# google/data-driven-discretization-1d

Hardware: AMD Instinct MI355X
Metric: grid-point-steps/s (higher is better)
Workload: dtype f32

## Files before the change

data-driven-discretization-1d_amd/csrc/rhs_mfma.h:

```cpp
#pragma once
#include <type_traits>
#include <utility>

#include "dev_params.h"
#include "mfma_layout.h"

namespace ddd {
namespace mfma {

constexpr int kHS = 36;
constexpr int kTrigMax = 12;
__host__ __device__ constexpr int tab_rows(bool wide) { return wide ? 4 : 4 + flavour_channels(false); }

typedef float f32x16 __attribute__((ext_vector_type(16)));
typedef float f32x4 __attribute__((ext_vector_type(4)));
typedef float f32x2 __attribute__((ext_vector_type(2)));

template <int kK_, int kCB_>
struct Tower {
  static constexpr int kK = kK_;
  static constexpr int kCB = kCB_;
  static constexpr int kC = 32 * kCB_;
  static constexpr int kHS = kC + 4;
  static constexpr int kInSteps = (kK_ + 2) / 2;
// ... 255 lines not shown
  const float t = __builtin_amdgcn_exp2f(ax * -2.885390081777927f);
  const float q = (1.0f - t) * __builtin_amdgcn_rcpf(1.0f + t);
  const float x2 = x * x;
  const float poly =
      ax * fmaf(x2, fmaf(x2, fmaf(x2, fmaf(x2, 62.0f / 2835.0f, -17.0f / 315.0f), 2.0f / 15.0f),
                         -1.0f / 3.0f), 1.0f);
  return copysignf(ax < 0.25f ? poly : q, x);
}

__device__ __forceinline__ void activate16(f32x16& acc, int act) {
  if (act == ACT_RELU) {
#pragma unroll
    for (int r = 0; r < 16; r += 2) {
      f32x2 v{acc[r], acc[r + 1]}, y;
      asm("v_pk_add_f32 %0, %1, 0 clamp" : "=v"(y) : "v"(v));
      acc[r] = y[0];
      acc[r + 1] = y[1];
    }
  } else if (act == ACT_RELU6) {
#pragma unroll
    for (int r = 0; r < 16; ++r) acc[r] = fminf(fmaxf(acc[r], 0.0f), 6.0f);
  } else if (act == ACT_TANH) {
#pragma unroll
    for (int r = 0; r < 16; ++r) acc[r] = fast_tanh(acc[r]);
  } else if (act == ACT_SOFTPLUS) {
#pragma unroll
    for (int r = 0; r < 16; ++r) acc[r] = apply_activation(acc[r], ACT_SOFTPLUS);
  } else if (act == ACT_ELU) {
#pragma unroll
    for (int r = 0; r < 16; ++r) acc[r] = apply_activation(acc[r], ACT_ELU);
  }
}

__device__ __forceinline__ void store_tile32(float* out, int trow, int half,
                                             const f32x16& acc) {
  float* orow = out + trow * kHS + 4 * half;
#pragma unroll
  for (int qd = 0; qd < 4; ++qd)
    *reinterpret_cast<float4*>(orow + 8 * qd) = make_float4(
        acc[4 * qd + 0], acc[4 * qd + 1], acc[4 * qd + 2], acc[4 * qd + 3]);
}

__device__ __forceinline__ void store_tile32_at_bytes(float* out, int byte_off, const f32x16& acc) {
  char* orow = reinterpret_cast<char*>(out) + byte_off;
#pragma unroll
  for (int qd = 0; qd < 4; ++qd)
    *reinterpret_cast<float4*>(orow + 32 * qd) = make_float4(
        acc[4 * qd + 0], acc[4 * qd + 1], acc[4 * qd + 2], acc[4 * qd + 3]);
}

__device__ __forceinline__ float upper_half_one(float x) {
  return __builtin_amdgcn_inverse_ballot_w64(0xffffffff00000000ull) ? 1.0f : x;
}

template <int kWR, bool kShfl, bool kAddr = false>
__device__ __forceinline__ void input_layer(const DevParams& p, const Lane& ln,
                                            const float* __restrict__ us, float un,
                                            float* __restrict__ out,
                                            const float (&w)[kInSteps],
                                            const int (&rows)[2][kKW], int act,
                                            const int (*bperm)[3] = nullptr, int st_off = 0) {
  constexpr int kT = kWR / 32;
  const int j = ln.lane & 31;
  const int half = ln.lane >> 5;
  f32x16 acc[kT];
  float b0[kT], b1[kT], b2[kT];
#pragma unroll
  for (int t = 0; t < kT; ++t) {
    if (kAddr && kShfl) {
      const int uni = __float_as_int(un);
      b0[t] = __int_as_float(__builtin_amdgcn_ds_bpermute(bperm[t][0], uni));
      b1[t] = __int_as_float(__builtin_amdgcn_ds_bpermute(bperm[t][1], uni));
      b2[t] = __int_as_float(__builtin_amdgcn_ds_bpermute(bperm[t][2], uni));
    } else if (kAddr) {
      const char* __restrict__ ub = reinterpret_cast<const char*>(us);
      b0[t] = *reinterpret_cast<const float*>(ub + bperm[t][0]);
      b1[t] = *reinterpret_cast<const float*>(ub + bperm[t][1]);
      b2[t] = *reinterpret_cast<const float*>(ub + bperm[t][2]);
    } else {
      const int r0 = half ? rows[t][1] : rows[t][0];
      const int r1 = half ? rows[t][3] : rows[t][2];
      const int r2 = rows[t][4];
      b0[t] = kShfl ? __shfl(un, r0, 64) : us[r0];
      b1[t] = kShfl ? __shfl(un, r1, 64) : us[r1];
      b2[t] = kShfl ? __shfl(un, r2, 64) : us[r2];
    }
    b2[t] = kAddr ? upper_half_one(b2[t]) : (half ? 1.0f : b2[t]);
  }
  if (kAddr && kShfl) __builtin_amdgcn_sched_group_barrier(0x080, 3 * kT, 0);
#pragma unroll
  for (int t = 0; t < kT; ++t) {
#pragma unroll
    for (int r = 0; r < 16; ++r) acc[t][r] = 0.0f;
  }
#pragma unroll
  for (int t = 0; t < kT; ++t) acc[t] = DDD_MFMA32(w[0], b0[t], acc[t]);
#pragma unroll
  for (int t = 0; t < kT; ++t) acc[t] = DDD_MFMA32(w[1], b1[t], acc[t]);
#pragma unroll
  for (int t = 0; t < kT; ++t) acc[t] = DDD_MFMA32(w[2], b2[t], acc[t]);
#pragma unroll
  for (int t = 0; t < kT; ++t) {
    activate16(acc[t], act);
    if (kAddr) store_tile32_at_bytes(out, st_off + t * 32 * kHS * 4, acc[t]);
    else store_tile32(out, ln.wave * kWR + t * 32 + j, half, acc[t]);
  }
}

template <int kWR, bool kByteOffsets = false, int kPrio = 0>
__device__ __forceinline__ void hidden_layer(const DevParams& p, const Lane& ln,
                                             const float* __restrict__ in,
                                             float* __restrict__ out,
                                             const float (&w)[kHidSteps],
                                             const int (&rows)[2][kKW], int act, int st_off = 0) {
  constexpr int kT = kWR / 32;
  const int j = ln.lane & 31;
  const int half = ln.lane >> 5;
  int rowo[kT][kKW];
#pragma unroll
  for (int t = 0; t < kT; ++t)
#pragma unroll
    for (int tap = 0; tap < kKW; ++tap)
      rowo[t][tap] = kByteOffsets ? rows[t][tap]
                                  : (int)__umul24((unsigned)rows[t][tap], (unsigned)(kHS * 4)) +
                                        64 * half;
  const auto operand = [&](int t, int tap, int q) {
    return *reinterpret_cast<const float4*>(reinterpret_cast<const char*>(in) + rowo[t][tap] + 16 * q);
  };
  f32x16 acc[kT];
  float4 cur[kT], nxt[kT];
#pragma unroll
  for (int t = 0; t < kT; ++t) {
#pragma unroll
    for (int r = 0; r < 16; ++r) acc[t][r] = 0.0f;
    cur[t] = operand(t, 0, 0);
  }
  __builtin_amdgcn_sched_group_barrier(0x100, kT, 0);
#pragma unroll
  for (int g = 0; g < 20; ++g) {
    if (kPrio == 5 && g == 1) __builtin_amdgcn_s_setprio(0);
    if (kPrio == 5 && g == 19) __builtin_amdgcn_s_setprio(3);
#pragma unroll
    for (int t = 0; t < kT; ++t) {
      nxt[t] = cur[t];
      if (g + 1 < 20) nxt[t] = operand(t, (g + 1) >> 2, (g + 1) & 3);
    }
#pragma unroll
    for (int t = 0; t < kT; ++t) acc[t] = DDD_MFMA32(w[4 * g + 0], cur[t].x, acc[t]);
#pragma unroll
    for (int t = 0; t < kT; ++t) acc[t] = DDD_MFMA32(w[4 * g + 1], cur[t].y, acc[t]);
#pragma unroll
    for (int t = 0; t < kT; ++t) acc[t] = DDD_MFMA32(w[4 * g + 2], cur[t].z, acc[t]);
#pragma unroll
    for (int t = 0; t < kT; ++t) acc[t] = DDD_MFMA32(w[4 * g + 3], cur[t].w, acc[t]);
#pragma unroll
    for (int t = 0; t < kT; ++t) cur[t] = nxt[t];
    __builtin_amdgcn_sched_group_barrier(0x100, kT, 0);
    __builtin_amdgcn_sched_group_barrier(0x008, 4 * kT, 0);
  }
#pragma unroll
  for (int t = 0; t < kT; ++t) {
    acc[t] = DDD_MFMA32(w[80], 1.0f, acc[t]);
  }
#pragma unroll
  for (int t = 0; t < kT; ++t) {
    activate16(acc[t], act);
    if (kByteOffsets) store_tile32_at_bytes(out, st_off + t * 32 * kHS * 4, acc[t]);
    else store_tile32(out, ln.wave * kWR + t * 32 + j, half, acc[t]);
  }
}

#define DDD_MFMA16(A, B, C) __builtin_amdgcn_mfma_f32_16x16x4f32((A), (B), (C), 0, 0, 0)
__host__ __device__ constexpr int quad_channel_float(int c) {
  return 4 * (4 * (c >> 4) + (c & 3)) + ((c & 15) >> 2);
}

__device__ __forceinline__ void activate4(f32x4& acc, int act) {
  if (act == ACT_RELU) {
#pragma unroll
    for (int r = 0; r < 4; r += 2) {
      f32x2 v{acc[r], acc[r + 1]}, y;
      asm("v_pk_add_f32 %0, %1, 0 clamp" : "=v"(y) : "v"(v));
      acc[r] = y[0];
      acc[r + 1] = y[1];
    }
  } else {
#pragma unroll
    for (int r = 0; r < 4; ++r) acc[r] = apply_activation(acc[r], act);
  }
}

__device__ __forceinline__ void store_tile16(float* out, int st_off, const f32x4& acc) {
  char* o = reinterpret_cast<char*>(out) + st_off;
#pragma unroll
  for (int r = 0; r < 4; ++r) *reinterpret_cast<float*>(o + 16 * r) = acc[r];
// ... 457 lines not shown
  }
#pragma unroll
  for (int h = 0; h < kCB; ++h)
#pragma unroll
    for (int t = 0; t < kT; ++t) acc[h][t] = DDD_MFMA32(wb[h], 1.0f, acc[h][t]);
#pragma unroll
  for (int h = 0; h < kCB; ++h)
#pragma unroll
    for (int t = 0; t < kT; ++t) {
      activate16(acc[h][t], act);
      store_tile32_at<TW::kHS>(out, ln.wave * kWR + t * 32 + j, h, half, acc[h][t]);
    }
}

template <int kAbid>
__device__ __forceinline__ f32x4 mfma4(float a, float b, f32x4 c) {
  return __builtin_amdgcn_mfma_f32_4x4x1f32(a, b, c, 4, kAbid, 0);
}

template <int NG, int Q0, int NW, int kAcc, int... J>
__device__ __forceinline__ void fin4_mfmas(const float (&w)[NW], const f32x4& b,
                                           f32x4 (&acc)[kAcc], std::integer_sequence<int, J...>) {
  ((acc[J % kAcc] = mfma4<(Q0 + J) % 16>(w[(Q0 + J) / 16], b[J / NG], acc[J % kAcc])), ...);
}

template <int NG>
__device__ __forceinline__ void load_final4(const DevParams& p, int lane,
                                            float (&w)[fin4_regs(NG)]) {
  load_rows4<fin4_regs(NG)>(p.w_final4, lane, w);
}

constexpr int kFin4Ahead = 2;

template <int NG, int OG, class TW, int kAcc>
__device__ __forceinline__ void fin4_step(const char* __restrict__ in, const int (&off)[TW::kK],
                                          const float (&w)[fin4_regs_t<TW>(NG)],
                                          f32x4 (&buf)[kFin4Ahead + 1], f32x4 (&acc)[kAcc]) {
  constexpr int kNext = OG + kFin4Ahead;
  constexpr int kPerTap = TW::kFinC / 4;
  if constexpr (kNext < TW::kOperandGroups)
    buf[kNext % (kFin4Ahead + 1)] =
        *reinterpret_cast<const f32x4*>(in + off[kNext / kPerTap] + 16 * (kNext % kPerTap));
  fin4_mfmas<NG, OG * 4 * NG, fin4_regs_t<TW>(NG), kAcc>(w, buf[OG % (kFin4Ahead + 1)], acc,
                                                         std::make_integer_sequence<int, 4 * NG>{});
  if constexpr (kNext < TW::kOperandGroups) __builtin_amdgcn_sched_group_barrier(0x100, 1, 0);
  __builtin_amdgcn_sched_group_barrier(0x008, 4 * NG, 0);
}

template <int NG, class TW, int kAcc, int... OG>
__device__ __forceinline__ void fin4_run(const char* __restrict__ in, const int (&off)[TW::kK],
                                         const float (&w)[fin4_regs_t<TW>(NG)],
                                         f32x4 (&buf)[kFin4Ahead + 1], f32x4 (&acc)[kAcc],
                                         std::integer_sequence<int, OG...>) {
  (fin4_step<NG, OG, TW, kAcc>(in, off, w, buf, acc), ...);
}

template <int NG, class TW = DefaultTower, int kAcc = NG, int kPrio = 0>
__device__ __forceinline__ void final_layer4(const float* __restrict__ in_f,
                                             const float (&w)[fin4_regs_t<TW>(NG)],
                                             const int (&off)[TW::kK], f32x4 (&acc)[kAcc]) {
  const char* __restrict__ in = reinterpret_cast<const char*>(in_f);
  constexpr int kPerTap = TW::kFinC / 4;
  f32x4 buf[kFin4Ahead + 1];
#pragma unroll
  for (int g = 0; g < kAcc; ++g) acc[g] = f32x4{0.0f, 0.0f, 0.0f, 0.0f};
#pragma unroll
  for (int og = 0; og < kFin4Ahead; ++og)
    buf[og] = *reinterpret_cast<const f32x4*>(in + off[og / kPerTap] + 16 * (og % kPerTap));
  __builtin_amdgcn_sched_group_barrier(0x100, kFin4Ahead, 0);
  if (kPrio == 5) __builtin_amdgcn_s_setprio(1);
  fin4_run<NG, TW, kAcc>(in, off, w, buf, acc, std::make_integer_sequence<int, TW::kOperandGroups>{});
  if (kPrio == 5) __builtin_amdgcn_s_setprio(3);
  fin4_mfmas<NG, (TW::kFinK - 1) * NG, fin4_regs_t<TW>(NG), kAcc>(
      w, f32x4{1.0f, 1.0f, 1.0f, 1.0f}, acc, std::make_integer_sequence<int, NG>{});
}

template <int NG, int kPrio = 0>
__device__ __forceinline__ void final_layer4_t16(const float* __restrict__ in_f,
                                                 const float (&w)[fin4_regs_t<Tile16Tower>(NG)],
                                                 const int (&off)[kKW], f32x4 (&acc)[NG]) {
  const char* __restrict__ in = reinterpret_cast<const char*>(in_f);
  f32x4 cur[4], nxt[4];
#pragma unroll
  for (int g = 0; g < NG; ++g) acc[g] = f32x4{0.0f, 0.0f, 0.0f, 0.0f};
#pragma unroll
  for (int q = 0; q < 4; ++q) cur[q] = *reinterpret_cast<const f32x4*>(in + off[0] + 16 * q);
  __builtin_amdgcn_sched_group_barrier(0x100, 4, 0);
  if (kPrio == 5) __builtin_amdgcn_s_setprio(1);
  constexpr int kNW = fin4_regs_t<Tile16Tower>(NG);
  const auto tap_steps = [&](auto tap_c) {
    constexpr int tap = decltype(tap_c)::value;
#pragma unroll
    for (int q = 0; q < 4; ++q) {
      nxt[q] = cur[q];
      if (tap + 1 < kKW) nxt[q] = *reinterpret_cast<const f32x4*>(in + off[tap + 1 < kKW ? tap + 1 : tap] + 16 * q);
    }
    fin4_mfmas<NG, (4 * tap + 0) * 4 * NG, kNW, NG>(w, f32x4{cur[0][0], cur[1][0], cur[2][0], cur[3][0]}, acc,
                                                 std::make_integer_sequence<int, 4 * NG>{});
    fin4_mfmas<NG, (4 * tap + 1) * 4 * NG, kNW, NG>(w, f32x4{cur[0][1], cur[1][1], cur[2][1], cur[3][1]}, acc,
                                                 std::make_integer_sequence<int, 4 * NG>{});
    fin4_mfmas<NG, (4 * tap + 2) * 4 * NG, kNW, NG>(w, f32x4{cur[0][2], cur[1][2], cur[2][2], cur[3][2]}, acc,
                                                 std::make_integer_sequence<int, 4 * NG>{});
    fin4_mfmas<NG, (4 * tap + 3) * 4 * NG, kNW, NG>(w, f32x4{cur[0][3], cur[1][3], cur[2][3], cur[3][3]}, acc,
                                                 std::make_integer_sequence<int, 4 * NG>{});
// ... 74 lines not shown
__device__ __forceinline__ void forcing_phase1(const DevParams& p, Shared<kRows, kWR, kWide, TW>& sm,
                                               const Resident& res, float t, int tid) {
  if (tid < res.frc_pairs) {
    float sn, cs;
    sincos_branchless(res.frc_omega * t + res.frc_phi, &sn, &cs);
    sm.pm[tid] = make_float2(res.frc_a * sn, res.frc_a * cs);
  }
}

template <int kRows, int kWR, bool kMasked = false, bool kWide = false, class TW = DefaultTower>
__device__ __forceinline__ float forcing_phase2(Shared<kRows, kWR, kWide, TW>& sm, const Resident& res) {
  const int cnt = (res.frc_run >> 16) & 0xff;
  const float* __restrict__ pm = reinterpret_cast<const float*>(sm.pm) + (res.frc_run & 0xffff);
  float acc = 0.0f;
  int first = 0;
  if (kMasked) {
    float v[8];
#pragma unroll
    for (int i = 0; i < 8; ++i) v[i] = pm[2 * i];
#pragma unroll
    for (int i = 0; i < 8; ++i) acc = fmaf(v[i], res.frc_mask[i], acc);
    first = 8;
  }
  for (int m = first; m < cnt; m += 8) {
    float v[8];
#pragma unroll
    for (int i = 0; i < 8; ++i) v[i] = pm[2 * (m + i)];
#pragma unroll
    for (int i = 0; i < 8; ++i) acc = acc + (m + i < cnt ? v[i] : 0.0f);
  }
  return acc;
}

template <int kRows, int kWR, bool kMasked = false, bool kWide = false, class TW = DefaultTower>
__device__ __forceinline__ float forcing_sums(const DevParams& p, Shared<kRows, kWR, kWide, TW>& sm,
                                              const Resident& res, float t, int tid) {
  forcing_phase1<kRows, kWR>(p, sm, res, t, tid);
  group_barrier<kRows, kWR>();
  return forcing_phase2<kRows, kWR, kMasked>(sm, res);
}

template <int kRows, int kWR, bool kHoist, int kEq, bool kTrace, bool kWide, class TW = DefaultTower>
__device__ __forceinline__ float eval_rhs(const DevParams& p, Shared<kRows, kWR, kWide, TW>& sm, int batch,
                                          float u, float t, float t_next, Resident& res,
                                          bool fast_forcing, float* derivs_out,
                                          float* coeffs_out, bool prepare_next = true,
                                          int group = -1, int ablate = 0,
                                          unsigned long long* trace = nullptr) {
#define DDD_STAMP(i) do { if (kTrace && trace != nullptr && group_tid<kRows, kWR>() == 0) trace[i] = __builtin_amdgcn_s_memtime(); } while (0)
  DDD_STAMP(0);
  constexpr bool kSpec = kEq >= 0;
  const int eqn = kSpec ? kEq : p.equation;
  const int nD = kSpec ? spec_derivs(kEq) : opaque_scalar(p.D);
  const int nG = kSpec ? spec_stencil(kEq) : opaque_scalar(p.G);
  const unsigned dsel_valid = kSpec ? 0u : (unsigned)opaque_scalar((int)p.dsel_valid);
  const unsigned long long dsel_bits = kSpec ? 0ull : opaque_scalar(p.dsel_bits);
  const int rt_groups = kSpec ? 0 : opaque_scalar(p.rt_groups);
  const bool flux_form = kSpec ? spec_flux_form(kEq) : (p.conservative != 0);
  const bool fixed = kSpec ? false : (p.fixed != 0 || p.linear_taps != 0);
  const bool folded = kSpec ? spec_folded(kSpec ? kEq : 0) : (p.folded != 0);
  const int target = kSpec ? (int)TARGET_COEFFICIENTS : p.target;
  const int act = kSpec ? (int)ACT_RELU : p.act;
  const bool forced = kSpec ? (spec_forced_family(kSpec ? kEq : 0) && p.forced != 0)
                            : (p.forced != 0);
  if (kSpec) fast_forcing = true;
  const int nL = kHoist ? 3 : p.L;
  const bool pow2 = kRows == 64 || (p.N & (p.N - 1)) == 0;
  constexpr bool kOneWave = kRows == kWR;
  constexpr int kPrio = prio_mode(kEq);
  constexpr int kNG = kSpec ? spec_fin_groups(kSpec ? kEq : 0) : 2;
  constexpr int kGW = flavour_stencil(kWide);
  constexpr int kCh = flavour_net_channels(kWide);
  static_assert(!(kSpec && kWide), "the per-equation kernels have no wide flavour");
  static_assert(TW::kDefault || (!kSpec && !kWide && !kHoist && kWR == 64),
                "towers other than 5 taps x 32 channels: run-time-parameterised kernels only");
  constexpr bool kSplit = kSpec && kRows == 64 && kWR == 32 && kHoist;
  constexpr bool kQuad = kSpec && kRows == 64 && kWR == 16 && kHoist;
  static_assert(kWR != 16 || kQuad, "16-row wavefronts: per-equation integrators only");
  constexpr bool kKeepOffsets = (kWR == 64 || kSplit || kQuad) && kHoist;
  constexpr bool kKeepRows = kKeepOffsets && kEq >= 0;
  constexpr bool kKeepPatch = kKeepOffsets && !kWide;
  const int tid = opaque(group_tid<kRows, kWR>());
  const Lane ln = make_lane<kRows, kWR>(p, batch, tid, group < 0 ? (int)blockIdx.x : group);
  if (ln.owner) sm.u[ln.row] = u;
  const bool clamps_nan = !fixed && (act == ACT_RELU || act == ACT_RELU6);
  if (clamps_nan && !kOneWave) {
    if (__builtin_amdgcn_ballot_w64(u != u) != 0 && ln.lane == 0) sm.nan_flag = 1;
  }
  const auto nan_in_receptive_field = [&]() -> bool {
    const int n = p.N, lk = p.K >> 1;
    int span = p.L * (p.K - 1);
    span = span < n - 1 ? span : n - 1;
    int q = (ln.pos - p.L * lk) % n;
    q = q < 0 ? q + n : q;
    bool hit = false;
    for (int i = 0; i <= span; ++i) {
      const float v = sm.u[ln.base + q];
      hit = hit || (v != v);
      q = q + 1 == n ? 0 : q + 1;
    }
    return hit;
  };
  int hid_rows[2][TW::kK];
  if (!fixed && !kQuad) {
    if constexpr (!TW::kDefault) {
#pragma unroll
      for (int t2 = 0; t2 < 2; ++t2)
        tap_rows_n<TW>(ln, ln.wave * kWR + t2 * 32 + (ln.lane & 31), p.N, pow2, hid_rows[t2]);
    } else if constexpr (kKeepOffsets) {
#pragma unroll
      for (int t2 = 0; t2 < 2; ++t2)
#pragma unroll
        for (int k = 0; k < kKW; ++k) hid_rows[t2][k] = res.hid_off[t2][k];
    } else {
// ... 2 lines not shown
        tap_rows<kRows == 64>(ln, ln.wave * kWR + t2 * 32 + (ln.lane & 31), p.N, hid_rows[t2]);
    }
  }
  const float q_un = u * p.inv_stddev;
  float un_reg = fmaf(fmaf(-q_un, p.stddev, u), p.inv_stddev, q_un);
  if (p.exact_div) {
    asm volatile("; exact division");
    un_reg = u / p.stddev;
  }
  if (!fixed && !kOneWave && ln.owner) sm.un[ln.row] = un_reg;
  group_barrier<kRows, kWR>();
  const bool trig_lds = p.n_k <= 4;
  if (forced && fast_forcing && res.frc_slot >= 0)
    sm.fk[res.frc_slot] = res.fk_next;

  bool nan_any = false, poisoned = false;
  if (clamps_nan && !kOneWave) {
    nan_any = __builtin_amdgcn_readfirstlane(sm.nan_flag) != 0;
    if (nan_any) poisoned = nan_in_receptive_field();
  }
  float pch[kGW];
  const int gl = nG >> 1;
  if (!kOneWave) {
#pragma unroll
    for (int g = 0; g < kGW; ++g)
      pch[g] = (g < nG) ? sm.u[kKeepPatch ? res.pch_idx[g < kGMax ? g : 0]
                               : pow2 ? (((ln.pos + g - gl) & (p.N - 1)) | ln.base)
                                      : wrap_row(ln.base, ln.pos, g - gl, p.N)] : 0.0f;
  }

  float net[kCh];
#pragma unroll
  for (int c = 0; c < kCh; ++c) net[c] = 0.0f;
  if (!fixed) {
    DDD_STAMP(1);
    if (kPrio) __builtin_amdgcn_s_setprio(kPrio == 2 ? 0 : 3);
    if constexpr (TW::kDefault && !kQuad) {
      if (!kHoist && nL > 2) load_hidden(p, 0, ln.lane, res.hid);
    }
    if constexpr (kQuad) {
      input_layer_quad(sm.un, sm.hA, res.q_in, res.q_in_off, res.q_st_off, act, ln.lane);
    } else if constexpr (TW::kTile16) {
      static_assert(kKeepOffsets && kWR == 64 && kOneWave, "16-channel tiles: resident one-wave integrators");
      input_layer_t16(un_reg, sm.hA, res.w_in, res.t16_in_perm, res.t16_st_off, act, ln.lane);
    } else if constexpr (!TW::kDefault) {
      input_layer_big<TW, kWR, kOneWave>(p, ln, sm.un, un_reg, sm.hA, hid_rows, act);
    } else if (!(ablate & 16)) {
      input_layer<kWR, kOneWave, kKeepOffsets>(p, ln, sm.un, un_reg, sm.hA, res.w_in, hid_rows,
                                               act, res.in_perm, res.st_off);
    }
    const bool frc_next = forced && fast_forcing && prepare_next && !(ablate & 1);
    if (frc_next) forcing_phase1<kRows, kWR>(p, sm, res, t_next, tid);
    float* in = sm.hA;
    float* out = Shared<kRows, kWR, kWide, TW>::kSingleBuffer ? sm.hA : sm.hB;
    for (int l = 1; l < nL - 1; ++l) {
      if constexpr (kQuad) {
        group_barrier<kRows, kWR>();
        hidden_layer_quad(in, out, res.q_hid, res.q_hid_off, res.q_st_off, act);
      } else if constexpr (!TW::kDefault) {
        group_barrier<kRows, kWR>();
        if constexpr (TW::kRolled)
          hidden_layer_rolled<TW, kWR>(p, ln, l - 1, in, out, p.N, pow2, act);
        else if (l == 1 && res.hw_valid)
          hidden_layer_stream<TW, kWR, resident_groups<TW>()>(p, ln, 0, in, out, hid_rows, act,
                                                              res.hw, res.hwb);
        else
          hidden_layer_stream<TW, kWR>(p, ln, l - 1, in, out, hid_rows, act);
      } else {
        if (!kHoist && l > 1) load_hidden(p, l - 1, ln.lane, res.hid);
        group_barrier<kRows, kWR>();
        if constexpr (TW::kTile16) {
          hidden_layer_t16<kPrio>(in, out, res.hid, res.t16_hid_off, res.t16_st_off, act);
        } else {
          hidden_layer<kWR, kKeepOffsets, kPrio>(p, ln, in, out, res.hid, hid_rows, act, res.st_off);
        }
      }
      float* tmp = in; in = out; out = tmp;
    }
    DDD_STAMP(2);
    {
      if constexpr (kQuad) {
        constexpr bool kMaskedSums = spec_folded(kSpec ? kEq : 0);
        if (frc_next) res.fk_next = forcing_phase2<kRows, kWR, kMaskedSums>(sm, res);
        group_barrier<kRows, kWR>();
        const f32x4 d4 = final_layer_quad(in, res.q_fin, res.q_fin_off);
        *reinterpret_cast<float4*>(reinterpret_cast<char*>(out) + res.q_xch_off) =
            make_float4(d4[0], d4[1], d4[2], d4[3]);
        asm volatile("s_waitcnt lgkmcnt(0)" ::: "memory");
        const float* mine = out + ln.row * kHS;
#pragma unroll
        for (int g4 = 0; g4 < kNG; ++g4) {
          const float4 v = *reinterpret_cast<const float4*>(mine + 4 * g4);
          net[4 * g4] = v.x; net[4 * g4 + 1] = v.y; net[4 * g4 + 2] = v.z; net[4 * g4 + 3] = v.w;
        }
      } else if constexpr (kSplit) {
        constexpr int kNA = (kNG + 1) / 2, kNB = kNG - kNA;
        constexpr bool kMaskedSums = spec_folded(kSpec ? kEq : 0);
        if (frc_next) res.fk_next = forcing_phase2<kRows, kWR, kMaskedSums>(sm, res);
        group_barrier<kRows, kWR>();
        int off4[kKW];
#pragma unroll
        for (int k = 0; k < kKW; ++k) off4[k] = res.fin4_off[k];
        float* xch = out + ln.lane * kHS;
        if (ln.wave == 0) {
          float wa[fin4_regs(kNA)];
#pragma unroll
          for (int s2 = 0; s2 < fin4_regs(kNA); ++s2) wa[s2] = res.w_fin4[s2];
// ... 26 lines not shown
      float wf4[kFirstRows];
      if (!kKeepRows) {
        if constexpr (kSpec) {
          load_rows4<kFirstRows>(p.w_final4, opaque(ln.lane), wf4);
        } else {
          const float* __restrict__ wsrc = p.w_final4_rt + opaque(ln.lane);
#pragma unroll
          for (int s2 = 0; s2 < kFirstRows; ++s2) wf4[s2] = wsrc[s2 * 64];
        }
      }
      int off4[TW::kK];
      if constexpr (kKeepRows) {
#pragma unroll
        for (int s2 = 0; s2 < kFirstRows; ++s2) wf4[s2] = res.w_fin4[s2];
      }
      if constexpr (!TW::kDefault) {
        int rows_k[TW::kK];
        tap_rows_n<TW>(ln, ln.row, p.N, pow2, rows_k);
#pragma unroll
        for (int k = 0; k < TW::kK; ++k)
          off4[k] = (int)__umul24((unsigned)rows_k[k], (unsigned)(TW::kHS * 4));
      } else if constexpr (kKeepOffsets) {
#pragma unroll
        for (int k = 0; k < kKW; ++k) off4[k] = res.fin4_off[k];
      } else {
        int rows5[kKW];
        tap_rows<kRows == 64>(ln, ln.row, p.N, rows5);
#pragma unroll
        for (int k = 0; k < kKW; ++k)
          off4[k] = (int)__umul24((unsigned)rows5[k], (unsigned)(kHS * 4));
      }
      if (nL == 2) group_barrier<kRows, kWR>();
      constexpr bool kMaskedSums = kKeepRows && spec_folded(kSpec ? kEq : 0);
      if (frc_next) res.fk_next = forcing_phase2<kRows, kWR, kMaskedSums>(sm, res);
      group_barrier<kRows, kWR>();
      if constexpr (kSpec) {
        f32x4 acc4[kNG];
        if (!(ablate & 4)) {
          if constexpr (TW::kTile16) final_layer4_t16<kNG, kPrio>(in, wf4, off4, acc4);
          else final_layer4<kNG, TW, kNG, kPrio>(in, wf4, off4, acc4);
        } else {
#pragma unroll
          for (int g4 = 0; g4 < kNG; ++g4) acc4[g4] = f32x4{0.0f, 0.0f, 0.0f, 0.0f};
        }
#pragma unroll
        for (int g4 = 0; g4 < kNG; ++g4)
#pragma unroll
          for (int r4 = 0; r4 < 4; ++r4) net[4 * g4 + r4] = acc4[g4][r4];
      } else if constexpr (!kSpec) {
        constexpr int kPairRows = fin4_regs_t<TW>(2);
        const int head = rt_head_groups(rt_groups);
        int done = 0;
        if (!(ablate & 4)) {
          float wnext[kPairRows];
          const auto fetch_pair = [&](int first_group) {
            const float* __restrict__ wn = p.w_final4_rt +
                (size_t)(fin4_regs_t<TW>(head) + (first_group - head) / 2 * kPairRows) * 64 +
                opaque(ln.lane);
#pragma unroll
            for (int s2 = 0; s2 < kPairRows; ++s2) wnext[s2] = wn[s2 * 64];
          };
          if (head > 0 && head < rt_groups) fetch_pair(head);
          if (head == 3) {
            f32x4 acc3[3];
            final_layer4<3, TW>(in, wf4, off4, acc3);
#pragma unroll
            for (int g4 = 0; g4 < 3; ++g4)
#pragma unroll
              for (int r4 = 0; r4 < 4; ++r4) net[4 * g4 + r4] = acc3[g4][r4];
          } else if (head == 1) {
            float w1[fin4_regs_t<TW>(1)];
#pragma unroll
            for (int s2 = 0; s2 < fin4_regs_t<TW>(1); ++s2) w1[s2] = wf4[s2];
            f32x4 acc1[2];
            final_layer4<1, TW, 2>(in, w1, off4, acc1);
#pragma unroll
// ... 42 lines not shown
    if (forced && fast_forcing && prepare_next && !(ablate & 1))
      res.fk_next = forcing_sums<kRows, kWR>(p, sm, res, t_next, tid);
    group_barrier<kRows, kWR>();
  }

  if (clamps_nan) {
    if (kOneWave) {
      nan_any = __builtin_amdgcn_ballot_w64(u != u) != 0;
      if (nan_any) poisoned = nan_in_receptive_field();
    }
    if (nan_any) {
      const float qnan = __int_as_float(0x7fc00000);
#pragma unroll
      for (int c = 0; c < kCh; ++c) net[c] = poisoned ? qnan : net[c];
    }
  }
  float4 trig4[kTrigMax / 4];
  if (forced && fast_forcing) {
    if (kKeepOffsets) {
#pragma unroll
      for (int i = 0; i < kTrigMax / 4; ++i) trig4[i] = res.trig[i];
    } else if (trig_lds) {
      trig4[0] = *reinterpret_cast<const float4*>(sm.hA + ln.row * TW::kHS + TW::kC);
      trig4[1] = *reinterpret_cast<const float4*>(
          sm.hB + ln.row * Shared<kRows, kWR, kWide, TW>::kHBStride + Shared<kRows, kWR, kWide, TW>::kHBPad);
      trig4[2] = make_float4(0.0f, 0.0f, 0.0f, 0.0f);
    } else {
      const float4* __restrict__ tr =
          reinterpret_cast<const float4*>(p.trig) + (size_t)opaque(ln.pos) * (kTrigMax / 4);
#pragma unroll
      for (int i = 0; i < kTrigMax / 4; ++i) trig4[i] = tr[i];
    }
  }
  if (kOneWave) {
#pragma unroll
    for (int g = 0; g < kGW; ++g)
      pch[g] = (g < nG) ? sm.u[kKeepPatch ? res.pch_idx[g < kGMax ? g : 0]
                               : pow2 ? (((ln.pos + g - gl) & (p.N - 1)) | ln.base)
                                      : wrap_row(ln.base, ln.pos, g - gl, p.N)] : 0.0f;
  }
  f32x2 cf2[kMaxDerivs][kGW / 2];
#define CF(d, g) cf2[d][(g) >> 1][(g) & 1]
#pragma unroll
  for (int d = 0; d < kMaxDerivs; ++d)
#pragma unroll
    for (int q = 0; q < kGW / 2; ++q) cf2[d][q] = f32x2{0.0f, 0.0f};
  if (kWide) {
    if (!fixed && target == TARGET_COEFFICIENTS) {
      const auto take = [&](auto slot_c) {
        constexpr int kSlot = decltype(slot_c)::value;
#pragma unroll
        for (int d = 0; d < kWideDerivs; ++d)
#pragma unroll
          for (int g = 0; g < kSlot; ++g)
            if (kSlot * d + g < kCh && g < kGW) CF(d, g) = net[(kSlot * d + g) % kCh];
      };
      if (nG <= kGMax) take(std::integral_constant<int, kGMax>{});
      else if (nG == 9) take(std::integral_constant<int, 9>{});
      else if (nG == 10) take(std::integral_constant<int, 10>{});
      else if (nG == 11) take(std::integral_constant<int, 11>{});
      else take(std::integral_constant<int, 12>{});
    }
  } else if (!fixed && folded) {
    if (kSpec) {
#pragma unroll
      for (int g = 0; g < kGW; ++g)
        if (g < nG) { CF(0, g) = net[g]; CF(1, g) = net[nG + g]; }
// ... 104 lines not shown
          s = fmaf(CF(d, g), pch[g], s);
          asm("" : "+v"(s));
        }
      dv[d] = s;
    }
  }
  if (derivs_out != nullptr && ln.active) {
#pragma unroll
    for (int d = 0; d < kMaxDerivs; ++d)
      if (d < nD) derivs_out[(size_t)ln.gidx * nD + d] = dv[d];
  }

  float r = equation_rhs_or_flux(eqn, u, dv, p.eta);
  const bool direct_time = !kSpec && !fixed && target == TARGET_TIME_DERIVATIVE;
  const bool direct_flux = !kSpec && !fixed && target == TARGET_FLUX;
  if (direct_time || direct_flux) r = net[0];
  if ((flux_form && !direct_time) || direct_flux) {
    float fnext;
    if (kOneWave) {
      if (p.N == 64 && p.dpp_rol)
        fnext = ops::wave_rotate_left1(r);
      else
        fnext = __shfl(r, pow2 ? (((ln.pos + 1) & (p.N - 1)) | ln.base)
                                    : wrap_row(ln.base, ln.pos, 1, p.N), 64);
    } else {
      if (ln.owner) sm.flux[ln.row] = r;
      group_barrier<kRows, kWR>();
      fnext = sm.flux[wrap_row(ln.base, ln.pos, 1, p.N)];
    }
    r = p.inv_dx * (fnext - r);
    if (!direct_flux) r = -r;
  }
  if (forced && !(ablate & 1)) {
    if (kSpec || fast_forcing) {
      const float4* __restrict__ fk4 =
          kKeepOffsets ? reinterpret_cast<const float4*>(reinterpret_cast<const char*>(sm.fk) + res.fk_off)
                       : reinterpret_cast<const float4*>(sm.fk + ln.sl * kTrigMax);
      float total = 0.0f;
#pragma unroll
      for (int i = 0; i < kTrigMax / 4; ++i) {
        if (i == 2 && trig_lds && !kKeepOffsets) break;
        const float4 f = fk4[i];
        total = fmaf(f.x, trig4[i].x, total);
        total = fmaf(f.y, trig4[i].y, total);
        total = fmaf(f.z, trig4[i].z, total);
        total = fmaf(f.w, trig4[i].w, total);
      }
      r = r + total;
    } else if (ln.valid) {
      r = r + forcing_at(p, p.frc + (size_t)(ln.gidx / p.N) * p.P, ln.pos, t);
    }
  }
  DDD_STAMP(4);
#undef DDD_STAMP
#undef CF
  return r;
}

template <int kRows, int kWR, bool kWide, class TW>
__device__ __forceinline__ void setup_samples(const DevParams& p, Shared<kRows, kWR, kWide, TW>& sm,
                                              int block, int batch, Resident& res, bool fast);

template <int kRows, int kWR>
__device__ __forceinline__ bool forcing_is_fast(const DevParams& p) {
  const int spg = kRows / p.N;
  return p.forced && spg * p.P <= Shared<kRows, kWR>::kPmMax && p.n_k <= 6 &&
         spg * kTrigMax <= Shared<kRows, kWR>::kFkMax && p.P < 256;
// ... 433 lines not shown
  const unsigned long long real0 = kTrace ? __builtin_amdgcn_s_memrealtime() : 0ull;
  const ST* y0 = static_cast<const ST*>(a.y0);
  ST* y_out = static_cast<ST*>(a.y_out);
  ST y = ln.valid ? y0[ln.gidx] : (ST)0;
  const ST h = (ST)a.dt;
  const size_t snap_stride = (size_t)a.batch * p.N;
  int until_save = a.save_every;
  size_t snap = 0;
  int evals = 0;
  if (fast_frc && !(ablate & 1))
    res.fk_next = forcing_sums<kRows, kWR>(p, sm, res, (float)(a.t0 + a.tab.c[0] * a.dt),
                                           (int)threadIdx.x);
  (void)h;
  constexpr bool kSgprStages = kEq >= 0;
  const StagePick<ST, kSgprStages> ah = stage_ah<ST, kSgprStages>(a.sc), bh = stage_bh<ST, kSgprStages>(a.sc);
  const StagePick<double, kSgprStages> ct(a.sc.ct);
  for (int step = 0; step < a.n_steps; ++step) {
    const double t = a.t0 + (double)step * a.dt;
    const double t_after = a.t0 + (double)(step + 1) * a.dt;
    ST ynew = y;
    float kprev = 0.0f;
    for (int s = 0; s < a.tab.stages; ++s) {
      ST us = y;
      if (s > 0) us = y + (ST)kprev * ah.at(s);
      unsigned long long* tr = nullptr;
      if (kTrace && trace_base != nullptr && evals * 5 + 5 <= kTraceSlots)
        tr = trace_base + (size_t)(int)blockIdx.x * kTraceSlots + evals * 5;
      ++evals;
      const bool last = s + 1 == a.tab.stages;
      const double tn = (last ? t_after : t) + ct.at(last ? 0 : s + 1);
      const float tn_lane = (float)tn;
      const float f = eval_rhs<kRows, kWR, kHoist, kEq, kTrace>(
          p, sm, a.batch, (float)us, (float)(t + ct.at(s)), tn_lane, res, fast_frc,
          nullptr, nullptr, true, -1, ablate, tr);
      if ((a.sc.b_nonzero >> s) & 1) ynew = ynew + bh.at(s) * (ST)f;
      kprev = f;
    }
    y = ynew;
    if (--until_save == 0) {
      until_save = a.save_every;
      if (ln.active) y_out[snap * snap_stride + ln.gidx] = y;
      ++snap;
    }
  }
  if (kTrace && trace_base != nullptr && threadIdx.x == 0) {
    unsigned long long* tr = trace_base + (size_t)blockIdx.x * kTraceSlots;
    tr[kTraceSlots - 2] = __builtin_amdgcn_s_memtime() - clk0;
    tr[kTraceSlots - 1] = __builtin_amdgcn_s_memrealtime() - real0;
  }
}

}
}
```

Measured before the change: 4.708 billion.

## Interleave epilogue and forcing LDS reads into final layer, use packed clamp activation

Adds an optional tail hook to the final 4x4 MFMA layer. It issues the stencil-patch, forcing-coefficient and forcing-phase2 LDS reads inside the MFMA operand stream, so their latency overlaps the matrix work instead of sitting after it. The forcing dot product and the first chunk of the next-step sums are computed right after the final layer and reused later. It also replaces the generic activation in the input and hidden layers with inline-asm packed adds using the clamp modifier, and moves the b2 select after a scheduling barrier. The clamp path ignores the runtime activation selector and clamps to [0,1], so it is only correct when the specialised equation's activation matches that; it also adds register pressure and scheduling constraints.

```diff
diff --git a/data-driven-discretization-1d_amd/csrc/rhs_mfma.h b/data-driven-discretization-1d_amd/csrc/rhs_mfma.h
--- a/data-driven-discretization-1d_amd/csrc/rhs_mfma.h
+++ b/data-driven-discretization-1d_amd/csrc/rhs_mfma.h
@@ -311,6 +311,42 @@
   }
 }
 
+template <bool kReuse>
+__device__ __forceinline__ void relu_clamp_fresh(f32x16& out, const f32x16& a) {
+  f32x2 y[8];
+#define DDD_PAIR(r) f32x2{a[2 * (r)], a[2 * (r) + 1]}
+  if constexpr (kReuse) {
+    const f32x16& a0 = out;
+#define DDD_PAIR0(r) f32x2{a0[2 * (r)], a0[2 * (r) + 1]}
+    asm("v_pk_add_f32 %0, %8, 0 clamp\n\tv_pk_add_f32 %1, %9, 0 clamp\n\t"
+        "v_pk_add_f32 %2, %10, 0 clamp\n\tv_pk_add_f32 %3, %11, 0 clamp\n\t"
+        "v_pk_add_f32 %4, %12, 0 clamp\n\tv_pk_add_f32 %5, %13, 0 clamp\n\t"
+        "v_pk_add_f32 %6, %14, 0 clamp\n\tv_pk_add_f32 %7, %15, 0 clamp"
+        : "=&v"(y[0]), "=&v"(y[1]), "=&v"(y[2]), "=&v"(y[3]), "=&v"(y[4]), "=&v"(y[5]),
+          "=&v"(y[6]), "=&v"(y[7])
+        : "v"(DDD_PAIR(0)), "v"(DDD_PAIR(1)), "v"(DDD_PAIR(2)), "v"(DDD_PAIR(3)),
+          "v"(DDD_PAIR(4)), "v"(DDD_PAIR(5)), "v"(DDD_PAIR(6)), "v"(DDD_PAIR(7)),
+          "v"(DDD_PAIR0(0)), "v"(DDD_PAIR0(1)), "v"(DDD_PAIR0(2)), "v"(DDD_PAIR0(3)),
+          "v"(DDD_PAIR0(4)), "v"(DDD_PAIR0(5)), "v"(DDD_PAIR0(6)), "v"(DDD_PAIR0(7)));
+#undef DDD_PAIR0
+  } else {
+    asm("v_pk_add_f32 %0, %8, 0 clamp\n\tv_pk_add_f32 %1, %9, 0 clamp\n\t"
+        "v_pk_add_f32 %2, %10, 0 clamp\n\tv_pk_add_f32 %3, %11, 0 clamp\n\t"
+        "v_pk_add_f32 %4, %12, 0 clamp\n\tv_pk_add_f32 %5, %13, 0 clamp\n\t"
+        "v_pk_add_f32 %6, %14, 0 clamp\n\tv_pk_add_f32 %7, %15, 0 clamp"
+        : "=&v"(y[0]), "=&v"(y[1]), "=&v"(y[2]), "=&v"(y[3]), "=&v"(y[4]), "=&v"(y[5]),
+          "=&v"(y[6]), "=&v"(y[7])
+        : "v"(DDD_PAIR(0)), "v"(DDD_PAIR(1)), "v"(DDD_PAIR(2)), "v"(DDD_PAIR(3)),
+          "v"(DDD_PAIR(4)), "v"(DDD_PAIR(5)), "v"(DDD_PAIR(6)), "v"(DDD_PAIR(7)));
+  }
+#undef DDD_PAIR
+#pragma unroll
+  for (int r = 0; r < 8; ++r) {
+    out[2 * r] = y[r][0];
+    out[2 * r + 1] = y[r][1];
+  }
+}
+
 __device__ __forceinline__ void store_tile32(float* out, int trow, int half,
                                              const f32x16& acc) {
   float* orow = out + trow * kHS + 4 * half;
@@ -332,7 +368,7 @@
   return __builtin_amdgcn_inverse_ballot_w64(0xffffffff00000000ull) ? 1.0f : x;
 }
 
-template <int kWR, bool kShfl, bool kAddr = false>
+template <int kWR, bool kShfl, bool kAddr = false, bool kFreshRelu = false>
 __device__ __forceinline__ void input_layer(const DevParams& p, const Lane& ln,
                                             const float* __restrict__ us, float un,
                                             float* __restrict__ out,
@@ -364,9 +400,10 @@
       b1[t] = kShfl ? __shfl(un, r1, 64) : us[r1];
       b2[t] = kShfl ? __shfl(un, r2, 64) : us[r2];
     }
-    b2[t] = kAddr ? upper_half_one(b2[t]) : (half ? 1.0f : b2[t]);
-  }
-  if (kAddr && kShfl) __builtin_amdgcn_sched_group_barrier(0x080, 3 * kT, 0);
+  }
+  if (kAddr && kShfl) __builtin_amdgcn_sched_barrier(0);
+#pragma unroll
+  for (int t = 0; t < kT; ++t) b2[t] = kAddr ? upper_half_one(b2[t]) : (half ? 1.0f : b2[t]);
 #pragma unroll
   for (int t = 0; t < kT; ++t) {
 #pragma unroll
@@ -378,6 +415,16 @@
   for (int t = 0; t < kT; ++t) acc[t] = DDD_MFMA32(w[1], b1[t], acc[t]);
 #pragma unroll
   for (int t = 0; t < kT; ++t) acc[t] = DDD_MFMA32(w[2], b2[t], acc[t]);
+  if constexpr (kFreshRelu) {
+    f32x16 y;
+    relu_clamp_fresh<false>(y, acc[0]);
+    store_tile32_at_bytes(out, st_off, y);
+    __builtin_amdgcn_sched_barrier(0);
+    y = acc[0];
+    relu_clamp_fresh<true>(y, acc[kT - 1]);
+    store_tile32_at_bytes(out, st_off + 32 * kHS * 4, y);
+    return;
+  }
 #pragma unroll
   for (int t = 0; t < kT; ++t) {
     activate16(acc[t], act);
@@ -386,7 +433,7 @@
   }
 }
 
-template <int kWR, bool kByteOffsets = false, int kPrio = 0>
+template <int kWR, bool kByteOffsets = false, int kPrio = 0, bool kFreshRelu = false>
 __device__ __forceinline__ void hidden_layer(const DevParams& p, const Lane& ln,
                                              const float* __restrict__ in,
                                              float* __restrict__ out,
@@ -440,6 +487,16 @@
 #pragma unroll
   for (int t = 0; t < kT; ++t) {
     acc[t] = DDD_MFMA32(w[80], 1.0f, acc[t]);
+  }
+  if constexpr (kFreshRelu) {
+    f32x16 y;
+    relu_clamp_fresh<false>(y, acc[0]);
+    store_tile32_at_bytes(out, st_off, y);
+    __builtin_amdgcn_sched_barrier(0);
+    y = acc[0];
+    relu_clamp_fresh<true>(y, acc[kT - 1]);
+    store_tile32_at_bytes(out, st_off + 32 * kHS * 4, y);
+    return;
   }
 #pragma unroll
   for (int t = 0; t < kT; ++t) {
@@ -963,12 +1020,35 @@
 
 constexpr int kFin4Ahead = 2;
 
-template <int NG, int OG, class TW, int kAcc>
+struct NoTail {
+  static constexpr int kHeadReads = 0, kReads = 0;
+  __device__ __forceinline__ void head() const {}
+  __device__ __forceinline__ void operator()() const {}
+};
+template <int kHeadN, class H, int kN, class F>
+struct Fin4Tail {
+  static constexpr int kHeadReads = kHeadN, kReads = kN;
+  const H& h;
+  const F& f;
+  __device__ __forceinline__ void head() const { h(); }
+  __device__ __forceinline__ void operator()() const { f(); }
+};
+constexpr int kFin4TailAt = 4, kFin4HeadAt = 1;
+template <int NG, int OG, class TW, int kAcc, class Tail>
 __device__ __forceinline__ void fin4_step(const char* __restrict__ in, const int (&off)[TW::kK],
                                           const float (&w)[fin4_regs_t<TW>(NG)],
-                                          f32x4 (&buf)[kFin4Ahead + 1], f32x4 (&acc)[kAcc]) {
+                                          f32x4 (&buf)[kFin4Ahead + 1], f32x4 (&acc)[kAcc],
+                                          const Tail& tail) {
   constexpr int kNext = OG + kFin4Ahead;
   constexpr int kPerTap = TW::kFinC / 4;
+  if constexpr (Tail::kHeadReads > 0 && OG == kFin4HeadAt) {
+    tail.head();
+    __builtin_amdgcn_sched_group_barrier(0x100, Tail::kHeadReads, 0);
+  }
+  if constexpr (Tail::kReads > 0 && OG == TW::kOperandGroups - kFin4TailAt) {
+    tail();
+    __builtin_amdgcn_sched_group_barrier(0x100, Tail::kReads, 0);
+  }
   if constexpr (kNext < TW::kOperandGroups)
     buf[kNext % (kFin4Ahead + 1)] =
         *reinterpret_cast<const f32x4*>(in + off[kNext / kPerTap] + 16 * (kNext % kPerTap));
@@ -978,18 +1058,19 @@
   __builtin_amdgcn_sched_group_barrier(0x008, 4 * NG, 0);
 }
 
-template <int NG, class TW, int kAcc, int... OG>
+template <int NG, class TW, int kAcc, class Tail, int... OG>
 __device__ __forceinline__ void fin4_run(const char* __restrict__ in, const int (&off)[TW::kK],
                                          const float (&w)[fin4_regs_t<TW>(NG)],
                                          f32x4 (&buf)[kFin4Ahead + 1], f32x4 (&acc)[kAcc],
-                                         std::integer_sequence<int, OG...>) {
-  (fin4_step<NG, OG, TW, kAcc>(in, off, w, buf, acc), ...);
-}
-
-template <int NG, class TW = DefaultTower, int kAcc = NG, int kPrio = 0>
+                                         const Tail& tail, std::integer_sequence<int, OG...>) {
+  (fin4_step<NG, OG, TW, kAcc>(in, off, w, buf, acc, tail), ...);
+}
+
+template <int NG, class TW = DefaultTower, int kAcc = NG, int kPrio = 0, class Tail = NoTail>
 __device__ __forceinline__ void final_layer4(const float* __restrict__ in_f,
                                              const float (&w)[fin4_regs_t<TW>(NG)],
-                                             const int (&off)[TW::kK], f32x4 (&acc)[kAcc]) {
+                                             const int (&off)[TW::kK], f32x4 (&acc)[kAcc],
+                                             const Tail& tail = Tail{}) {
   const char* __restrict__ in = reinterpret_cast<const char*>(in_f);
   constexpr int kPerTap = TW::kFinC / 4;
   f32x4 buf[kFin4Ahead + 1];
@@ -1000,7 +1081,8 @@
     buf[og] = *reinterpret_cast<const f32x4*>(in + off[og / kPerTap] + 16 * (og % kPerTap));
   __builtin_amdgcn_sched_group_barrier(0x100, kFin4Ahead, 0);
   if (kPrio == 5) __builtin_amdgcn_s_setprio(1);
-  fin4_run<NG, TW, kAcc>(in, off, w, buf, acc, std::make_integer_sequence<int, TW::kOperandGroups>{});
+  fin4_run<NG, TW, kAcc>(in, off, w, buf, acc, tail,
+                         std::make_integer_sequence<int, TW::kOperandGroups>{});
   if (kPrio == 5) __builtin_amdgcn_s_setprio(3);
   fin4_mfmas<NG, (TW::kFinK - 1) * NG, fin4_regs_t<TW>(NG), kAcc>(
       w, f32x4{1.0f, 1.0f, 1.0f, 1.0f}, acc, std::make_integer_sequence<int, NG>{});
@@ -1141,6 +1223,39 @@
   return acc;
 }
 
+template <int kRows, int kWR, bool kWide, class TW>
+__device__ __forceinline__ void forcing_phase2_reads(Shared<kRows, kWR, kWide, TW>& sm, const Resident& res,
+                                                     float (&v)[8]) {
+  const float* __restrict__ pm = reinterpret_cast<const float*>(sm.pm) + (res.frc_run & 0xffff);
+#pragma unroll
+  for (int i = 0; i < 8; ++i) v[i] = pm[2 * i];
+}
+template <bool kMasked>
+__device__ __forceinline__ float forcing_phase2_first(const Resident& res, const float (&v)[8]) {
+  const int cnt = (res.frc_run >> 16) & 0xff;
+  float acc = 0.0f;
+#pragma unroll
+  for (int i = 0; i < 8; ++i) {
+    if (kMasked) acc = fmaf(v[i], res.frc_mask[i], acc);
+    else acc = acc + (i < cnt ? v[i] : 0.0f);
+  }
+  return acc;
+}
+template <int kRows, int kWR, bool kWide, class TW>
+__device__ __forceinline__ float forcing_phase2_rest(Shared<kRows, kWR, kWide, TW>& sm, const Resident& res,
+                                                     float acc) {
+  const int cnt = (res.frc_run >> 16) & 0xff;
+  const float* __restrict__ pm = reinterpret_cast<const float*>(sm.pm) + (res.frc_run & 0xffff);
+  for (int m = 8; m < cnt; m += 8) {
+    float v[8];
+#pragma unroll
+    for (int i = 0; i < 8; ++i) v[i] = pm[2 * (m + i)];
+#pragma unroll
+    for (int i = 0; i < 8; ++i) acc = acc + (m + i < cnt ? v[i] : 0.0f);
+  }
+  return acc;
+}
+
 template <int kRows, int kWR, bool kMasked = false, bool kWide = false, class TW = DefaultTower>
 __device__ __forceinline__ float forcing_sums(const DevParams& p, Shared<kRows, kWR, kWide, TW>& sm,
                                               const Resident& res, float t, int tid) {
@@ -1149,13 +1264,15 @@
   return forcing_phase2<kRows, kWR, kMasked>(sm, res);
 }
 
-template <int kRows, int kWR, bool kHoist, int kEq, bool kTrace, bool kWide, class TW = DefaultTower>
+template <int kRows, int kWR, bool kHoist, int kEq, bool kTrace, bool kWide, class TW = DefaultTower,
+          bool kStreamSums = false>
 __device__ __forceinline__ float eval_rhs(const DevParams& p, Shared<kRows, kWR, kWide, TW>& sm, int batch,
                                           float u, float t, float t_next, Resident& res,
                                           bool fast_forcing, float* derivs_out,
                                           float* coeffs_out, bool prepare_next = true,
                                           int group = -1, int ablate = 0,
-                                          unsigned long long* trace = nullptr) {
+                                          unsigned long long* trace = nullptr,
+                                          std::integral_constant<bool, kStreamSums> = {}) {
 #define DDD_STAMP(i) do { if (kTrace && trace != nullptr && group_tid<kRows, kWR>() == 0) trace[i] = __builtin_amdgcn_s_memtime(); } while (0)
   DDD_STAMP(0);
   constexpr bool kSpec = kEq >= 0;
@@ -1189,6 +1306,8 @@
   constexpr bool kKeepOffsets = (kWR == 64 || kSplit || kQuad) && kHoist;
   constexpr bool kKeepRows = kKeepOffsets && kEq >= 0;
   constexpr bool kKeepPatch = kKeepOffsets && !kWide;
+  constexpr bool kFreshRelu = kKeepRows && kOneWave && kWR == 64 && TW::kDefault && !TW::kTile16;
+  constexpr bool kEarlyEpilogue = kFreshRelu;
   const int tid = opaque(group_tid<kRows, kWR>());
   const Lane ln = make_lane<kRows, kWR>(p, batch, tid, group < 0 ? (int)blockIdx.x : group);
   if (ln.owner) sm.u[ln.row] = u;
@@ -1257,6 +1376,7 @@
   float net[kCh];
 #pragma unroll
   for (int c = 0; c < kCh; ++c) net[c] = 0.0f;
+  float total_early = 0.0f;
   if (!fixed) {
     DDD_STAMP(1);
     if (kPrio) __builtin_amdgcn_s_setprio(kPrio == 2 ? 0 : 3);
@@ -1271,7 +1391,7 @@
     } else if constexpr (!TW::kDefault) {
       input_layer_big<TW, kWR, kOneWave>(p, ln, sm.un, un_reg, sm.hA, hid_rows, act);
     } else if (!(ablate & 16)) {
-      input_layer<kWR, kOneWave, kKeepOffsets>(p, ln, sm.un, un_reg, sm.hA, res.w_in, hid_rows,
+      input_layer<kWR, kOneWave, kKeepOffsets, kFreshRelu>(p, ln, sm.un, un_reg, sm.hA, res.w_in, hid_rows,
                                                act, res.in_perm, res.st_off);
     }
     const bool frc_next = forced && fast_forcing && prepare_next && !(ablate & 1);
@@ -1297,7 +1417,7 @@
         if constexpr (TW::kTile16) {
           hidden_layer_t16<kPrio>(in, out, res.hid, res.t16_hid_off, res.t16_st_off, act);
         } else {
-          hidden_layer<kWR, kKeepOffsets, kPrio>(p, ln, in, out, res.hid, hid_rows, act, res.st_off);
+          hidden_layer<kWR, kKeepOffsets, kPrio, kFreshRelu>(p, ln, in, out, res.hid, hid_rows, act, res.st_off);
         }
       }
       float* tmp = in; in = out; out = tmp;
@@ -1390,16 +1510,60 @@
       }
       if (nL == 2) group_barrier<kRows, kWR>();
       constexpr bool kMaskedSums = kKeepRows && spec_folded(kSpec ? kEq : 0);
-      if (frc_next) res.fk_next = forcing_phase2<kRows, kWR, kMaskedSums>(sm, res);
+      constexpr bool kEarlySums = kEarlyEpilogue && kStreamSums && kMaskedSums &&
+                                  spec_forced_family(kSpec ? kEq : 0);
+      if (!kEarlySums && frc_next) res.fk_next = forcing_phase2<kRows, kWR, kMaskedSums>(sm, res);
       group_barrier<kRows, kWR>();
       if constexpr (kSpec) {
         f32x4 acc4[kNG];
+        constexpr bool kSums = kEarlyEpilogue && spec_forced_family(kSpec ? kEq : 0);
+        float4 fk_early[kTrigMax / 4];
+        const auto epilogue_reads = [&]() {
+          if constexpr (kEarlyEpilogue) {
+#pragma unroll
+            for (int g = 0; g < kGW; ++g) pch[g] = (g < nG) ? sm.u[res.pch_idx[g < kGMax ? g : 0]] : 0.0f;
+            if constexpr (kSums) {
+              const float4* __restrict__ fk4 = reinterpret_cast<const float4*>(
+                  reinterpret_cast<const char*>(sm.fk) + res.fk_off);
+#pragma unroll
+              for (int i = 0; i < kTrigMax / 4; ++i) fk_early[i] = fk4[i];
+            }
+          }
+        };
+        constexpr int kTailReads =
+            kEarlyEpilogue ? spec_stencil(kSpec ? kEq : 0) + (kSums ? kTrigMax / 4 : 0) : 0;
+        float pm_early[8];
+        const auto phase2_reads = [&]() {
+          if constexpr (kEarlySums) forcing_phase2_reads(sm, res, pm_early);
+        };
+        const Fin4Tail<(kEarlySums ? 4 : 0), decltype(phase2_reads), kTailReads, decltype(epilogue_reads)>
+            tail{phase2_reads, epilogue_reads};
         if (!(ablate & 4)) {
           if constexpr (TW::kTile16) final_layer4_t16<kNG, kPrio>(in, wf4, off4, acc4);
-          else final_layer4<kNG, TW, kNG, kPrio>(in, wf4, off4, acc4);
+          else final_layer4<kNG, TW, kNG, kPrio>(in, wf4, off4, acc4, tail);
         } else {
 #pragma unroll
           for (int g4 = 0; g4 < kNG; ++g4) acc4[g4] = f32x4{0.0f, 0.0f, 0.0f, 0.0f};
+          tail.head();
+          tail();
+        }
+        float sum_next = 0.0f;
+        if constexpr (kEarlySums) {
+          sum_next = forcing_phase2_first<kMaskedSums>(res, pm_early);
+          asm volatile("" : "+v"(sum_next));
+        }
+        if constexpr (kSums) {
+#pragma unroll
+          for (int i = 0; i < kTrigMax / 4; ++i) {
+            total_early = fmaf(fk_early[i].x, res.trig[i].x, total_early);
+            total_early = fmaf(fk_early[i].y, res.trig[i].y, total_early);
+            total_early = fmaf(fk_early[i].z, res.trig[i].z, total_early);
+            total_early = fmaf(fk_early[i].w, res.trig[i].w, total_early);
+          }
+          asm volatile("" : "+v"(total_early));
+          if constexpr (kEarlySums) {
+            if (frc_next) res.fk_next = forcing_phase2_rest(sm, res, sum_next);
+          }
         }
 #pragma unroll
         for (int g4 = 0; g4 < kNG; ++g4)
@@ -1508,7 +1672,7 @@
       for (int i = 0; i < kTrigMax / 4; ++i) trig4[i] = tr[i];
     }
   }
-  if (kOneWave) {
+  if (kOneWave && (!kEarlyEpilogue || fixed)) {
 #pragma unroll
     for (int g = 0; g < kGW; ++g)
       pch[g] = (g < nG) ? sm.u[kKeepPatch ? res.pch_idx[g < kGMax ? g : 0]
@@ -1679,7 +1843,9 @@
     if (!direct_flux) r = -r;
   }
   if (forced && !(ablate & 1)) {
-    if (kSpec || fast_forcing) {
+    if (kEarlyEpilogue && !fixed) {
+      r = r + total_early;
+    } else if (kSpec || fast_forcing) {
       const float4* __restrict__ fk4 =
           kKeepOffsets ? reinterpret_cast<const float4*>(reinterpret_cast<const char*>(sm.fk) + res.fk_off)
                        : reinterpret_cast<const float4*>(sm.fk + ln.sl * kTrigMax);
@@ -2179,7 +2345,7 @@
       const float tn_lane = (float)tn;
       const float f = eval_rhs<kRows, kWR, kHoist, kEq, kTrace>(
           p, sm, a.batch, (float)us, (float)(t + ct.at(s)), tn_lane, res, fast_frc,
-          nullptr, nullptr, true, -1, ablate, tr);
+          nullptr, nullptr, true, -1, ablate, tr, std::true_type{});
       if ((a.sc.b_nonzero >> s) & 1) ynew = ynew + bh.at(s) * (ST)f;
       kprev = f;
     }
```

Result: faster. 4.791 billion, median of 6 (+1.7%).
